# huyhoang17/DB_text_minimal

Hardware: AMD Instinct MI355X
Metric: train images/sec @640x640 bs=16/GPU (higher is better)
Workload: dtype f32

## Files before the change

db_text_minimal_amd/_lib.py:

```python
import ctypes
import os
import subprocess

_HERE = os.path.dirname(os.path.abspath(__file__))
LIB_PATH = os.environ.get('DBN_LIB_PATH') or os.path.join(_HERE, 'libdbnet_hip.so')
CSRC = os.path.join(_HERE, 'csrc')

_P, _I, _L, _F = ctypes.c_void_p, ctypes.c_int, ctypes.c_long, ctypes.c_float

SIGNATURES = {
    'dbn_pack_weights': 'piiiiiipp',
    'dbn_igemm_panel_floats': 'iiiiii',
    'dbn_igemm_packed_floats': 'ii',
    'dbn_igemm_f32': 'pppp' + 'i' * 14 + 'p',
    'dbn_igemm_tile_config': 'ii',
    'dbn_igemm_tile_config_ns': 'iii',
    'dbn_conv_bn_ws_floats': 'iiiiii',
    'dbn_pack_weights_batched': 'piip',
    'dbn_igemm_splitk_plan': 'iiii',
    'dbn_igemm_splitk_plan_ns': 'iiiii',
    'dbn_igemm_splitk_f32': 'pppp' + 'i' * 16 + 'pp',
    'dbn_deform_im2col': 'ppp' + 'i' * 11 + 'p',
    'dbn_deform_col2im': 'ppppp' + 'i' + 'p' + 'i' * 11 + 'p',
    'dbn_deform_col2im_ws_bytes': 'i' * 8,
# ... 82 lines not shown
    'dbn_db_loss_fwd': 'pp' + 'iiii' + 'ffff' + 'pppp',
    'dbn_db_loss_sum_fwd': 'pp' + 'iiii' + 'ffff' + 'pppp',
    'dbn_db_loss_frac_fwd': 'pp' + 'iiii' + 'ffff' + 'i' + 'pppp',
    'dbn_db_loss_bwd': 'pppp' + 'ff' + 'iiii' + 'pp',
    'dbn_db_loss_ohem_ws_bytes': 'iii',
    'dbn_db_loss_ohem_fwd': 'pp' + 'iiii' + 'ffff' + 'pppp',
    'dbn_db_loss_ohem_bwd': 'ppppp' + 'ff' + 'iiii' + 'pp',
    'dbn_pixel_confusion': 'plppiiifpp',
    'dbn_adam_step': 'pppp' + 'l' + 'ffff' + 'i' + 'f' + 'p',
    'dbn_clock_probe': 'pip',
    'dbn_has_experiments': '',
    'dbn_wall_clock_khz': '',
}
SIGNATURES.update({
    'dbn_igemm_t': 'ii' + 'pppp' + 'i' * 14 + 'i' + 'p' + 'p',
    'dbn_conv_bn_t': 'i' + SIGNATURES['dbn_conv_bn_f32'],
    'dbn_pyramid_conv_t': 'i' + SIGNATURES['dbn_pyramid_conv_f32'],
    'dbn_pyramid_conv_from_t': 'ii' + SIGNATURES['dbn_pyramid_conv_f32'],
    'dbn_igemm_bn_rows': 'i' * 15,
    'dbn_igemm_bnsums_t': 'ii' + 'pppp' + 'i' * 14 + 'ppppppp' + 'pppp' + 'p' + 'p',
    'dbn_igemm_bn_final_counters': 'ii',
    'dbn_igemm_bn_final_group_floats': 'ii',
    'dbn_wgrad_t': 'ii' + 'pppp' + 'i' * 12 + 'f' + 'p',
    'dbn_wgrad_phase_t': 'iii' + 'pppp' + 'i' * 12 + 'f' + 'p',
    'dbn_wgrad_reduce_describe': 'ii' + 'pppp' + 'i' * 12 + 'f' + 'p',
    'dbn_wgrad_reduce_many': 'ppiiip',
    'dbn_wgrad_tile_config': 'ii',
    'dbn_set_wgrad_variant': 'i',
    'dbn_set_convt_kernel': 'i',
    'dbn_igemm_splitk_slab_floats': 'iiiii',
    'dbn_wgrad_kernel_config': 'iiiii',
    'dbn_wgrad_kernel_config_hw': 'i' * 12,
    'dbn_set_patch_conv': 'i',
    'dbn_set_wres16': 'i',
    'dbn_set_pyramid_wide': 'i',
    'dbn_pyramid_wide_would_run': 'iiiiii',
    'dbn_conv_bn_set_final': 'pp',
    'dbn_conv_bn_final_group_doubles': 'ii',
    'dbn_wres16_would_run': 'iiiiiiiii',
    'dbn_mfma_sustained': 'ippip',
    'dbn_mfma_sustained_flops': 'ii',
    'dbn_set_stagger': 'i',
    'dbn_winograd_eligible': 'iiiii',
    'dbn_winograd_panel_floats': 'ii',
    'dbn_winograd_pack': 'piiiipp',
    'dbn_winograd_rows': 'iii',
    'dbn_winograd_pack_batched': 'pip',
    'dbn_winograd_dgrad_bnsums_f32': 'ppp' + 'iiiiii' + 'pppp' + 'ppp' + 'pppp' + 'p' + 'p',
    'dbn_winograd_ws_floats': 'iiii',
    'dbn_winograd_wgrad_eligible': 'iiiiii',
    'dbn_winograd_wgrad_linear': 'ii',
    'dbn_winograd_wgrad_slab_floats': 'iiiii',
    'dbn_winograd_wgrad_f32': 'ipppppp' + 'iiiiii' + 'fp',
    'dbn_winograd_conv_bn_act_f32': 'pppppp' + 'iiiii' + 'pp' + 'ff' + 'ppppppp' + 'p',
    'dbn_winograd_conv_bn_f32': 'pppp' + 'iiiii' + 'pp' + 'ff' + 'ppppppp' + 'p',
    'dbn_set_phase_priority': 'i',
    'dbn_set_winograd_persistent': 'i',
    'dbn_set_winograd_stagger': 'i',
    'dbn_set_winograd_blocks_per_barrier': 'i',
    'dbn_fold_bn_eval': 'pilppppp' + 'f' + 'ppp',
    'dbn_igemm_act_t': 'ii' + 'pppp' + 'i' + 'p' + 'i' * 13 + 'p',
    'dbn_winograd_conv_act_f32': 'pppp' + 'i' + 'p' + 'iiiii' + 'p',
    'dbn_pyramid_conv_act_t': 'ii' + 'p' * 9 + 'i' + 'p' + 'i' * 6 + 'p',
    'dbn_set_trace': 'pl',
    'dbn_igemm_kernel_config': 'i' * 16,
    'dbn_split3': 'pplp',
    'dbn_deform_im2col_t': 'i' + SIGNATURES['dbn_deform_im2col'],
    'dbn_deform_col2im_t': 'i' + SIGNATURES['dbn_deform_col2im'],
    'dbn_deform_col2im_gather_t': 'i' + SIGNATURES['dbn_deform_col2im'],
    'dbn_deform_col2im_gather_ws_bytes': 'iii',
    'dbn_deform_offset_absmax_t': 'iplpp',
    'dbn_pw16_eligible': 'iiiiii',
    'dbn_pw16_panel_bytes': '',
    'dbn_pw16_pack': 'ipipp',
    'dbn_pw16_act_t': 'ipppipiiiip',
    'dbn_set_head_tail_wide': 'i',
    'dbn_stem16_pool_eligible': 'iiii',
    'dbn_stem16_conv_bn_relu_pool_t': 'ipppppiiip',
    'dbn_head16_eligible': 'iiii',
    'dbn_head16_tail_eval_t': 'i' + 'p' * 15 + 'iii' + 'p',
    'dbn_cast_f32': 'ipplp',
    'dbn_pack_weights_t': 'ip' + 'i' * 7 + 'pp',
    'dbn_igemm_panel_floats_t': 'i' * 8,
    'dbn_bn_train_stats_t': 'i' + SIGNATURES['dbn_bn_train_stats'],
    'dbn_bn_apply_t': 'i' + SIGNATURES['dbn_bn_apply'],
    'dbn_bn_backward_t': 'ipi' + SIGNATURES['dbn_bn_backward_ex'][1:],
    'dbn_col_sum_t': 'i' + SIGNATURES['dbn_col_sum'],
    'dbn_bnrelu_maxpool_fwd_t': 'i' + SIGNATURES['dbn_bnrelu_maxpool_fwd'],
    'dbn_bnrelu_maxpool_bwd_t': 'i' + SIGNATURES['dbn_bnrelu_maxpool_bwd'][:-1] + 'pppp',
    'dbn_maxpool_bwd_parts': 'iiii',
    'dbn_bnrelu_maxpool_fwd_arg_t': 'ipppppp' + 'iiii' + 'p',
    'dbn_maxpool_bn_backward_ws_floats': 'iiii',
    'dbn_maxpool_bn_backward_t': 'i' + 'p' * 10 + 'iiii' + 'f' + 'pp',
    'dbn_nearest_up_fwd_t': 'i' + SIGNATURES['dbn_nearest_up_fwd'],
    'dbn_nearest_up_bwd_t': 'i' + SIGNATURES['dbn_nearest_up_bwd'],
    'dbn_nchw3_to_nhwc4_t': 'i' + SIGNATURES['dbn_nchw3_to_nhwc4'],
    'dbn_nchw3_to_nhwc4_packed_t': 'i' + SIGNATURES['dbn_nchw3_to_nhwc4'],
    'dbn_nchw3_to_nhwc16_and_4_t': 'ipppiiip',
    'dbn_convt16_rows': '',
    'dbn_convt16_panel_bytes': '',
    'dbn_convt16_eligible': 'iiiiii',
    'dbn_convt16_pack': 'ippp',
    'dbn_convt16_bn_t': 'ippppiii' + 'pp' + 'ff' + 'ppppppp' + 'p',
    'dbn_stem16_padded_h': 'i',
    'dbn_stem16_padded_w': 'i',
    'dbn_stem16_rows': '',
# ... 74 lines not shown
```

db_text_minimal_amd/csrc/wgrad.hip:

```cpp
#include "wgrad_kernels.h"

namespace {

constexpr int WRG = 16;
__global__ __launch_bounds__(256) void wgrad_reduce_kernel(const float* __restrict__ slab, int splitk, int O, int J, int Jp, int BM, int BN,
                                                           int Cb, int I, int R, int S, float* __restrict__ grad, float scale, int natural) {
    __shared__ double part[WRG][16][4];
    const long total = (long)O * Jp, count4 = total >> 2, total4 = wgrad_slab_stride(O, Jp) >> 2;
    const int pos = threadIdx.x & 15, g = threadIdx.x >> 4;
    const long q = blockIdx.x * 16L + pos;
    double s[4] = {0.0, 0.0, 0.0, 0.0};
    if (q < count4) {
        const f32x4* src = reinterpret_cast<const f32x4*>(slab) + q;
        int z = g;
        for (; z + 3 * WRG < splitk; z += 4 * WRG) {
            const f32x4 v0 = src[(long)z * total4], v1 = src[(long)(z + WRG) * total4];
            const f32x4 v2 = src[(long)(z + 2 * WRG) * total4], v3 = src[(long)(z + 3 * WRG) * total4];
#pragma unroll
            for (int e = 0; e < 4; ++e) s[e] += ((double)v0[e] + (double)v1[e]) + ((double)v2[e] + (double)v3[e]);
        }
        for (; z < splitk; z += WRG) {
            const f32x4 v = src[(long)z * total4];
#pragma unroll
            for (int e = 0; e < 4; ++e) s[e] += (double)v[e];
// ... 295 lines not shown
        size_t smem;
        wgrad_reduce64_plan(R * S, splits_total, G, threads, smem);
        *reduce_job = WgradReduceJob{slab, grad_oihw, splits_total, O, J, Jp, bm, bn, Cb, I, R * S, G, natural ? 1 : 0, O * (Cb / 64), scale,
                                     (int)smem};
        return DBN_OK;
    }
    if (Cb % 64 == 0 && R * S * 64 * 4 <= 32 * 1024) {
        int G, threads;
        size_t smem;
        wgrad_reduce64_plan(R * S, splits_total, G, threads, smem);
        hipLaunchKernelGGL(wgrad_reduce64_kernel, dim3(O, Cb / 64), dim3(threads), smem, st, slab, splits_total, O, J, Jp, bm, bn, Cb, I,
                           R * S, G, grad_oihw, scale, natural ? 1 : 0);
    } else
        hipLaunchKernelGGL(wgrad_reduce_kernel, dim3((unsigned)(((long)O * Jp / 4 + 15) / 16)), dim3(256), 0, st, slab, splits_total, O, J, Jp, bm, bn,
                           Cb, I, R, S, grad_oihw, scale, natural ? 1 : 0);
    return dbn_status();
}

int dbn_wgrad_t(int at, int ns, const void* sm, const void* big, float* slab, float* grad_oihw, int N, int Ho, int Wo, int O, int H, int W,
                int Cb, int I, int R, int S, int stride, int pad, float scale, void* stream) {
    return wgrad_run(sm, big, slab, grad_oihw, N, Ho, Wo, O, H, W, Cb, I, R, S, stride, pad, scale, ns, stream, at);
}
int dbn_wgrad_phase_t(int phase, int at, int ns, const void* sm, const void* big, float* slab, float* grad_oihw, int N, int Ho, int Wo,
                      int O, int H, int W, int Cb, int I, int R, int S, int stride, int pad, float scale, void* stream) {
    DBN_REQUIRE(phase == 1 || phase == 2);
    return wgrad_run(sm, big, slab, grad_oihw, N, Ho, Wo, O, H, W, Cb, I, R, S, stride, pad, scale, ns, stream, at, phase);
}

int dbn_wgrad_reduce_describe(int at, int ns, const void* sm, const void* big, float* slab, float* grad_oihw, int N, int Ho, int Wo, int O,
                              int H, int W, int Cb, int I, int R, int S, int stride, int pad, float scale, void* job) {
    DBN_REQUIRE(job);
    return wgrad_run(sm, big, slab, grad_oihw, N, Ho, Wo, O, H, W, Cb, I, R, S, stride, pad, scale, ns, nullptr, at, 2,
                     reinterpret_cast<WgradReduceJob*>(job));
}
int dbn_wgrad_reduce_many(const void* jobs, const int* first, int n_jobs, int total_blocks, int max_smem, void* stream) {
    DBN_REQUIRE(jobs && first && n_jobs > 0 && total_blocks > 0 && max_smem > 0 && max_smem <= 64 * 1024);
    hipLaunchKernelGGL(wgrad_reduce64_many_kernel, dim3(total_blocks), dim3(1024), (size_t)max_smem, (hipStream_t)stream,
                       reinterpret_cast<const WgradReduceJob*>(jobs), first, n_jobs);
    return dbn_status();
}

int dbn_wgrad_f32(const float* sm, const float* big, float* slab, float* grad_oihw, int N, int Ho, int Wo, int O, int H, int W,
                  int Cb, int I, int R, int S, int stride, int pad, float scale, void* stream) {
    return wgrad_run(sm, big, slab, grad_oihw, N, Ho, Wo, O, H, W, Cb, I, R, S, stride, pad, scale, 0, stream);
}

int dbn_wgrad_bf16s(const float* sm, const float* big, float* slab, float* grad_oihw, int N, int Ho, int Wo, int O, int H, int W,
                    int Cb, int I, int R, int S, int stride, int pad, float scale, int ns, void* stream) {
    DBN_REQUIRE(ns == 1 || ns == 3);
    return wgrad_run(sm, big, slab, grad_oihw, N, Ho, Wo, O, H, W, Cb, I, R, S, stride, pad, scale, ns, stream);
}

}
```

db_text_minimal_amd/csrc/wgrad_kernels.h:

```cpp
#pragma once
#include "igemm_common.h"

struct WgradParams {
    const void* sm;
    const void* big;
    float* slab;
    int N, Ho, Wo, O, H, W, Cb, R, S, stride, pad;
    int P, J, pchunk;
    float rcp_HWo, rcp_Wo;
    unsigned sm_bytes, big_bytes;
    unsigned sm_plane_bytes, big_plane_bytes;
    int row_tw;
};

static inline int wgrad_row_tw(int Ho, int Wo) { return Wo % 16 == 0 ? 16 : (Wo % 8 == 0 && Ho % 2 == 0) ? 8 : (Wo % 4 == 0 && Ho % 4 == 0) ? 4 : 0; }

#ifndef DBN_DBG
#define DBN_DBG 0
#endif

namespace {

__host__ __device__ inline long wgrad_slab_stride(long O, long Jp) { return O * Jp + 1088; }


__host__ __device__ __forceinline__ int tile_pos_to_index(int pos, int B) { return 4 * (pos % (B / 4)) + pos / (B / 4); }

template <int BM, int BN, int WM, int WN, int NS, int AT = 0, int ROW = 0>
__global__ __launch_bounds__(WM* WN * 64) void wgrad_f32_kernel(const WgradParams p) {
    static_assert(AT == 0 || (AT == 1 && NS == 1) || (AT == 3 && NS == 3), "storage type / matrix math combination");
    static_assert(!ROW || AT == 0, "scalar-offset addressing is built for fp32 storage");
    constexpr unsigned ES = AT == 0 ? 4u : 2u;
    constexpr int NP = AT == 3 ? 3 : 1;
    constexpr int NT = WM * WN * 64;
    constexpr int TM = BM / WM, TN = BN / WN;
    constexpr int MI = TM / 32, NI = TN / 32;
    constexpr int AS = NS == 0 ? BM + 2 : BM + 4, BS = NS == 0 ? BN + 2 : BN + 4;
    constexpr int A_IMG = NS == 0 ? 4 * AS : NS * 2 * AS, B_IMG = NS == 0 ? 4 * BS : NS * 2 * BS;
    constexpr int STAGE = A_IMG + B_IMG;
    constexpr int NSX = NS > 0 ? NS : 1;
    static_assert(BM + BN <= NT && BM % 64 == 0 && BN % 64 == 0, "staging roles must fit the workgroup in whole waves");
    __shared__ f32x4 smem[2 * STAGE];

    const int tid = threadIdx.x;
    const int lane = tid & 63, wave = tid >> 6;
    const int wm = wave / WN, wn = wave % WN;
    const int li = lane & 31, lh = lane >> 5;

    const int njt = (p.J + BN - 1) / BN;
    const int ntiles = (p.O / BM) * njt;
    const int work = dbn_xcd_remap(blockIdx.x, gridDim.x);
    const int split = work / ntiles, tile_ = work - split * ntiles;
    const int ot = tile_ / njt, jt = tile_ - ot * njt;
    const int o0 = ot * BM, j0 = jt * BN;
    const int pbeg = (DBN_DBG & 8) ? 0 : split * p.pchunk;
    const int pend = min(p.P, pbeg + p.pchunk);
    const int KT = (pend - pbeg + 15) / 16;

    const __amdgpu_buffer_rsrc_t rs_sm = __builtin_amdgcn_make_buffer_rsrc(const_cast<void*>(p.sm), 0, p.sm_bytes, 0x00020000);
    const unsigned row_shift = ROW ? (unsigned)((p.pad * p.W + p.pad) * p.Cb) * ES : 0u;
    const __amdgpu_buffer_rsrc_t rs_big = __builtin_amdgcn_make_buffer_rsrc(
        const_cast<char*>(reinterpret_cast<const char*>(p.big) - row_shift), 0, p.big_bytes + row_shift, 0x00020000);

    const int wave_first = __builtin_amdgcn_readfirstlane(tid) & ~63;
    const bool is_a = wave_first < BM;
    const bool is_b = wave_first >= NT - BN;
    const int slot = is_a ? tid : tid - (NT - BN);
    const int qn = is_a ? BM / 4 : BN / 4;
    const int s_c = slot % qn, s_g = slot / qn;
    const int jj = j0 + 4 * s_c;
    const bool j_ok = is_b && jj < p.J;
    const int tap = j_ok ? jj / p.Cb : 0;
    const int ci = j_ok ? jj - tap * p.Cb : 0;
    const int tr = tap / p.S - p.pad, ts = (DBN_DBG & 16) ? 0 : tap % p.S - p.pad;
    const int HWo = p.Ho * p.Wo;
    const int ld = is_a ? AS : BS;
    const int lds_base = (is_a ? 0 : A_IMG) + s_c;

    constexpr int D = AT == 3 ? 1 : NS == 0 ? ((BM == 64 || ROW) ? 2 : 1) : (AT == 0 ? 3 : 4);
    f32x4 rr_[D][4];
    u32x2 rh_[D][NP][4];
    unsigned woff[4] = {OOB_OFFSET, OOB_OFFSET, OOB_OFFSET, OOB_OFFSET};
    int w_n, w_oh, w_ow;
    {
        int rem;
        divmod24(pbeg + 4 * s_g, HWo, p.rcp_HWo, w_n, rem);
        divmod24(rem, p.Wo, p.rcp_Wo, w_oh, w_ow);
    }
    unsigned vcon[4] = {OOB_OFFSET, OOB_OFFSET, OOB_OFFSET, OOB_OFFSET};
    int ccol[4] = {0, 0, 0, 0};
    int crow = 0;
    int s_n = 0, s_oh = 0, s_ow = 0;
    unsigned soff = 0;
    const int TW = ROW ? p.row_tw : 16, TH = 16 / TW;
    if constexpr (ROW) {
        const bool live = KT > 0;
        const int qy = (4 * s_g) / TW;
        crow = qy * p.stride + tr;
#pragma unroll
        for (int i = 0; i < 4; ++i) {
            const int qx = (4 * s_g + i) & (TW - 1);
            if (is_a) {
                vcon[i] = live ? (unsigned)((qy * p.Wo + qx) * p.O + o0 + 4 * s_c) * ES : OOB_OFFSET;
                woff[i] = vcon[i];
            } else if (is_b) {
                ccol[i] = qx * p.stride + ts;
                vcon[i] = (live && j_ok) ? row_shift + (unsigned)((crow * p.W + ccol[i]) * p.Cb + ci) * ES : OOB_OFFSET;
            }
        }
        const int bw = p.Wo / TW, bh = p.Ho / TH;
        const int t0 = __builtin_amdgcn_readfirstlane(pbeg >> 4);
        const int r0 = t0 / bw;
        s_ow = (t0 - r0 * bw) * TW;
        s_n = r0 / bh;
        s_oh = (r0 - s_n * bh) * TH;
// ... 214 lines not shown
    auto step = [&](int kt, auto UU) {
        constexpr int U = decltype(UU)::value;
        const int buf = kt & 1;
        offsets(kt + D);
        issue_loads(UU);
        const f32x4* As = smem + buf * STAGE;
        const f32x4* Bs = As + A_IMG;
        if constexpr (NS == 0) {
            f32x4 af[2][MI], bf[2][NI];
#pragma unroll
            for (int s2 = 0; s2 < 2; ++s2) {
#pragma unroll
                for (int a = 0; a < MI; ++a) af[s2][a] = As[(2 * s2 + lh) * AS + wm * TM + a * 32 + li];
#pragma unroll
                for (int b = 0; b < NI; ++b) bf[s2][b] = Bs[(2 * s2 + lh) * BS + wn * TN + b * 32 + li];
            }
#pragma unroll
            for (int s2 = 0; s2 < 2; ++s2)
#pragma unroll
                for (int e = 0; e < 4; ++e)
#pragma unroll
                    for (int a = 0; a < MI; ++a)
#pragma unroll
                        for (int b = 0; b < NI; ++b)
                            acc[a][b] = __builtin_amdgcn_mfma_f32_32x32x2f32(af[s2][a][e], bf[s2][b][e], acc[a][b], 0, 0, 0);
        } else {
            bf16x8 af[NSX][MI], bf[NSX][NI];
#pragma unroll
            for (int t = 0; t < NS; ++t) {
#pragma unroll
                for (int a = 0; a < MI; ++a) af[t][a] = __builtin_bit_cast(bf16x8, As[(t * 2 + lh) * AS + wm * TM + a * 32 + li]);
#pragma unroll
                for (int b = 0; b < NI; ++b) bf[t][b] = __builtin_bit_cast(bf16x8, Bs[(t * 2 + lh) * BS + wn * TN + b * 32 + li]);
            }
            mfma_split<NS, MI, NI>(af, bf, acc);
        }
        stage(buf ^ 1, std::integral_constant<int, (U + 1) % D>{});
        __syncthreads();
    };
    static_assert(D <= 4, "the k-loop spells the sets out");
    int kt = 0;
    for (; kt + D <= KT; kt += D) {
        step(kt, std::integral_constant<int, 0>{});
        if constexpr (D > 1) step(kt + 1, std::integral_constant<int, 1 % D>{});
        if constexpr (D > 2) step(kt + 2, std::integral_constant<int, 2 % D>{});
        if constexpr (D > 3) step(kt + 3, std::integral_constant<int, 3 % D>{});
    }
    if (kt < KT) step(kt, std::integral_constant<int, 0>{});
    if (D > 2 && kt + 1 < KT) step(kt + 1, std::integral_constant<int, 1 % D>{});
    if (D > 3 && kt + 2 < KT) step(kt + 2, std::integral_constant<int, 2 % D>{});
    }

    const int Jp = njt * BN;
    float* out = p.slab + (long)split * wgrad_slab_stride(p.O, Jp);
#pragma unroll
    for (int a = 0; a < MI; ++a)
#pragma unroll
        for (int b = 0; b < NI; ++b) {
            const int col = j0 + wn * TN + b * 32 + li;
#pragma unroll
            for (int r = 0; r < 16; ++r) {
                const int row = o0 + wm * TM + a * 32 + (r & 3) + 8 * (r >> 2) + 4 * lh;
                out[(long)row * Jp + col] = acc[a][b][r];
            }
        }
}

#if DBN_HAS_EXPERIMENTS
template <int BM, int BN, int WM, int WN>
__global__ __launch_bounds__(256) void wgrad_dma_kernel(const WgradParams p) {
    constexpr int KP = 16;
    constexpr int TM = BM / WM, TN = BN / WN, MI = TM / 32, NI = TN / 32;
    constexpr int A_F4 = KP * BM / 4, B_F4 = KP * BN / 4;
    constexpr int A_INSTR = A_F4 / 64, B_INSTR = B_F4 / 64;
    constexpr int PER_WAVE = (A_INSTR + B_INSTR) / 4;
    static_assert((A_INSTR + B_INSTR) % 4 == 0 && WM * WN == 4, "DMA instructions are dealt to four waves");
    constexpr int NSTG = 3;
    constexpr int STAGE_F4 = A_F4 + B_F4;
    __shared__ f32x4 smem[NSTG * STAGE_F4];

    const int tid = threadIdx.x;
    const int lane = tid & 63;
    const int wave = __builtin_amdgcn_readfirstlane(tid >> 6);
    const int wm = wave / WN, wn = wave % WN;
    const int li = lane & 31, lh = lane >> 5;

    const int njt = (p.J + BN - 1) / BN;
    const int ntiles = (p.O / BM) * njt;
    const int work = dbn_xcd_remap(blockIdx.x, gridDim.x);
    const int split = work / ntiles, tile_ = work - split * ntiles;
    const int ot = tile_ / njt, jt = tile_ - ot * njt;
    const int o0 = ot * BM, j0 = jt * BN;
    const int pbeg = split * p.pchunk;
    const int pend = min(p.P, pbeg + p.pchunk);
    const int KT = (pend - pbeg + KP - 1) / KP;

    const __amdgpu_buffer_rsrc_t rs_sm = __builtin_amdgcn_make_buffer_rsrc(const_cast<void*>(p.sm), 0, p.sm_bytes, 0x00020000);
    const __amdgpu_buffer_rsrc_t rs_big = __builtin_amdgcn_make_buffer_rsrc(const_cast<void*>(p.big), 0, p.big_bytes, 0x00020000);

    const int HWo = p.Ho * p.Wo;
    unsigned a_off[PER_WAVE];
    int a_px[PER_WAVE];
    int b_n[PER_WAVE], b_oh[PER_WAVE], b_ow[PER_WAVE], b_px[PER_WAVE], b_ci[PER_WAVE], b_tr[PER_WAVE], b_ts[PER_WAVE];
    bool b_ok[PER_WAVE];
#pragma unroll
    for (int i = 0; i < PER_WAVE; ++i) {
        const int t = wave * PER_WAVE + i;
// ... 405 lines not shown
#pragma unroll
                    for (int b = 0; b < 3; ++b) asm volatile("" : "+v"(fb[t][b][h2]));
                }
            typedef unsigned u32x4_ __attribute__((ext_vector_type(4)));
            bf16x8 af[NS][1], bf[NS][3];
#pragma unroll
            for (int t = 0; t < NS; ++t) {
                af[t][0] = __builtin_bit_cast(bf16x8, u32x4_{fa[t][0][0], fa[t][0][1], fa[t][1][0], fa[t][1][1]});
#pragma unroll
                for (int b = 0; b < 3; ++b)
                    bf[t][b] = __builtin_bit_cast(bf16x8, u32x4_{fb[t][b][0][0], fb[t][b][0][1], fb[t][b][1][0], fb[t][b][1][1]});
            }
            f32x16 (&acc2)[1][3] = reinterpret_cast<f32x16 (&)[1][3]>(acc);
            mfma_split<NS, 1, 3>(af, bf, acc2);
        });
    }

    float* out = p.slab + (long)split * wgrad_slab_stride(p.O, p.J);
#pragma unroll
    for (int b = 0; b < 3; ++b) {
        const int cblk = 3 * wn + b, s_ = cblk >> 1, half = cblk & 1;
        const int col = (3 * r + s_) * p.Cb + ci0 + 32 * half + li;
#pragma unroll
        for (int e = 0; e < 16; ++e) {
            const int row = o0 + 32 * wm + (e & 3) + 8 * (e >> 2) + 4 * lh;
            out[(long)row * p.J + col] = acc[b][e];
        }
    }
}

template <int NS, int AT, int ROW>
int launch_wgrad_tiles_row(const WgradParams& p, int bm, int bn, dim3 grid, hipStream_t st) {
    if (bn == 192)
        hipLaunchKernelGGL((wgrad_f32_kernel<64, 192, 2, 2, NS, AT, ROW>), grid, dim3(256), 0, st, p);
    else if (bm == 128 && bn == 128)
        hipLaunchKernelGGL((wgrad_f32_kernel<128, 128, 2, 2, NS, AT, ROW>), grid, dim3(256), 0, st, p);
    else if (bn == 128)
        hipLaunchKernelGGL((wgrad_f32_kernel<64, 128, 2, 2, NS, AT, ROW>), grid, dim3(256), 0, st, p);
    else
        hipLaunchKernelGGL((wgrad_f32_kernel<64, 64, 2, 2, NS, AT, ROW>), grid, dim3(256), 0, st, p);
    return dbn_status();
}
template <int NS, int AT>
int launch_wgrad_tiles(const WgradParams& p, int bm, int bn, dim3 grid, hipStream_t st) {
    if constexpr (AT == 0)
        if (p.row_tw && p.pchunk % 16 == 0) return launch_wgrad_tiles_row<NS, AT, 1>(p, bm, bn, grid, st);
    return launch_wgrad_tiles_row<NS, AT, 0>(p, bm, bn, grid, st);
}

}

int dbn_launch_wgrad_f32(const WgradParams& p, int kind, int bm, int bn, dim3 grid, hipStream_t st);
int dbn_launch_wgrad_b16(const WgradParams& p, int kind, int ns, int at, int bm, int bn, dim3 grid, hipStream_t st);
```

db_text_minimal_amd/csrc/winograd_wgrad_f32.hip:

```cpp
#include "igemm_common.h"
#include <algorithm>
#ifndef DBN_WWG_PIPE
#define DBN_WWG_PIPE 1
#endif
#ifndef DBN_WWG_EXP
#define DBN_WWG_EXP 0
#endif

namespace {

constexpr int WG_XPX = 180, WG_XROW = 18, WG_YPX = 128, WG_YROW = 16;

struct WinoWgradParams {
    const float* x;
    const float* dy;
    float* slab;
    int N, H, W, Cx, Cy;
    int nob, nib;
    int tw, gpi, groups;
    int nsplit;
    unsigned x_bytes, dy_bytes;
    const float *x_scale, *x_shift;
};

constexpr int WL_XPX = 336, WL_YPX = 240;
template <bool LIN>
__global__ __launch_bounds__(512) __attribute__((amdgpu_waves_per_eu(2, 2))) void winograd_wgrad_f32_kernel(const WinoWgradParams p) {
    constexpr int XPX = LIN ? WL_XPX : WG_XPX, YPX = LIN ? WL_YPX : WG_YPX;
    constexpr int XCH = XPX * 16, YCH = YPX * 16;
    constexpr int NXP = (XCH + 511) / 512, NYP = (YCH + 511) / 512;
    constexpr int NBUF = LIN ? 1 : 2;
    __shared__ f32x4 smem[NBUF * (XCH + YCH)];
    const int tid = threadIdx.x, lane = tid & 63, wave = __builtin_amdgcn_readfirstlane(tid >> 6);
    const int li = lane & 31, lh = lane >> 5;
    const int irow = wave & 3, oh = wave >> 2;
    const int nsub = p.nob * p.nib;
    const int b = dbn_xcd_remap(blockIdx.x, gridDim.x);
    const int split = b / nsub, sub = b - split * nsub;
    const int ob = sub / p.nib, ib = sub - ob * p.nib;
    const int g0 = (int)((long)split * p.groups / p.nsplit), g1 = (int)((long)(split + 1) * p.groups / p.nsplit);
    const __amdgpu_buffer_rsrc_t rsX = __builtin_amdgcn_make_buffer_rsrc(const_cast<float*>(p.x), 0, p.x_bytes, 0x00020000);
    const __amdgpu_buffer_rsrc_t rsY = __builtin_amdgcn_make_buffer_rsrc(const_cast<float*>(p.dy), 0, p.dy_bytes, 0x00020000);
    const int TW = (p.W + 1) >> 1, TI = ((p.H + 1) >> 1) * TW;
    const int prow = LIN ? 2 * TW + 2 : WG_XROW, yrow = LIN ? 2 * TW : WG_YROW;
    const float rTW = 1.0f / (float)TW;

    unsigned xrel[NXP], yrel[NYP];
    int xpos[NXP], ypos[NYP];
#pragma unroll
    for (int j = 0; j < NXP; ++j) {
        const int idx = tid + j * 512, pix = idx >> 4, ch = idx & 15;
        int py, px;
        if constexpr (LIN) divmod24(pix, prow, 1.0f / (float)prow, py, px);
// ... 327 lines not shown
    for (int pt = 0; pt < 16; ++pt)
#pragma unroll
        for (int e = 0; e < 4; ++e) acc[pt][e] = 0.0;
    for (int z = z0; z < z1; ++z) {
        f32x4 v[16];
#pragma unroll
        for (int pt = 0; pt < 16; ++pt) v[pt] = *reinterpret_cast<const f32x4*>(src + z * stride + pt * 4096);
#pragma unroll
        for (int pt = 0; pt < 16; ++pt)
#pragma unroll
            for (int e = 0; e < 4; ++e) acc[pt][e] += (double)v[pt][e];
    }
    if (zl2 >= ZH) {
#pragma unroll
        for (int pt = 0; pt < 16; ++pt)
#pragma unroll
            for (int e = 0; e < 4; ++e) part[zl * OG + og][pt][iq * 4 + e] = acc[pt][e];
    }
    __syncthreads();
    if (zl2 < ZH) {
#pragma unroll
        for (int pt = 0; pt < 16; ++pt)
#pragma unroll
            for (int e = 0; e < 4; ++e) part[zl * OG + og][pt][iq * 4 + e] += acc[pt][e];
    }
    __syncthreads();
    for (int k = threadIdx.x; k < OG * 16 * 32; k += 256) {
        const int g = k >> 9, pt = (k >> 5) & 15, c = k & 31;
        double s_ = 0.0;
#pragma unroll
        for (int q = 0; q < ZH; ++q) s_ += part[q * OG + g][pt][c];
        sh[g][pt][c] = s_;
    }
    __syncthreads();
    for (int k = threadIdx.x; k < OG * 288; k += 256) {
        const int g = k / 288, kk = k - g * 288, c = kk / 9, tap = kk - c * 9, r = tap / 3, q = tap - r * 3;
        auto gcol = [](int w, double v0, double v1, double v2, double v3) {
            return w == 0 ? v0 + 0.5 * (v1 + v2) : (w == 1 ? 0.5 * (v1 - v2) : 0.5 * (v1 + v2) + v3);
        };
        double t[4];
#pragma unroll
        for (int i = 0; i < 4; ++i) t[i] = gcol(q, sh[g][4 * i + 0][c], sh[g][4 * i + 1][c], sh[g][4 * i + 2][c], sh[g][4 * i + 3][c]);
        st[k] = (float)(gcol(r, t[0], t[1], t[2], t[3]) * (double)scale);
    }
    __syncthreads();
    const int c0 = ib * 64 + ih * 32;
    const int n = max(0, min(32, I - c0)) * 9;
    for (int k = threadIdx.x; k < OG * n; k += 256) {
        const int g = k / n, kk = k - g * n;
        grad[((long)(blockIdx.x * OG + g) * I + c0) * 9 + kk] = st[g * 288 + kk];
    }
}

int wwg_splits(int groups, int nsub) {
    static const int wgs = dbn_env_int("DBN_WWG_WGS", 256);
    int ns = std::max(1, wgs / nsub);
    return std::min(ns, groups);
}

bool wwg_linear_fits(int H, int W) {
    const int TW = (W + 1) / 2, TH = (H + 1) / 2;
    const int R = std::min(TH, (30 + TW) / TW + 1);
    return (2 * R + 2) * (2 * TW + 2) <= WL_XPX && 2 * R * 2 * TW <= WL_YPX;
}
double wwg_fill(int H, int W, bool lin) {
    if (lin) {
        const long TI = (long)((H + 1) / 2) * ((W + 1) / 2);
        return (double)TI / (double)((TI + 31) / 32 * 32);
    }
    return (double)H * W / ((double)((H + 7) / 8 * 8) * ((W + 15) / 16 * 16));
}
bool wwg_linear(int H, int W) {
    static const int env = dbn_env_int("DBN_WWG_LIN", 1);
    return env && wwg_linear_fits(H, W) && wwg_fill(H, W, true) > wwg_fill(H, W, false) + 0.2;
}
int wwg_groups(int N, int H, int W) {
    if (wwg_linear(H, W)) return N * (int)(((long)((H + 1) / 2) * ((W + 1) / 2) + 31) / 32);
    return N * ((H + 7) / 8) * ((W + 15) / 16);
}

}

extern "C" {

int dbn_winograd_wgrad_eligible(int N, int H, int W, int O, int Cb, int I) {
    if (N < 1 || H < 1 || W < 1 || O % 64 || Cb % 64 || I < 1 || I > Cb) return 0;
    const long px = (long)N * H * W;
    if (px * std::max(O, Cb) * 4 >= dbn_g_byte_limit) return 0;
    return wwg_fill(H, W, wwg_linear(H, W)) >= 0.5;
}
int dbn_winograd_wgrad_linear(int H, int W) { return wwg_linear(H, W); }
long dbn_winograd_wgrad_slab_floats(int N, int H, int W, int O, int Cb) {
    const int nsub = (O / 64) * (Cb / 64);
    return (long)wwg_splits(wwg_groups(N, H, W), nsub) * nsub * 16 * 4096;
}
int dbn_winograd_wgrad_f32(int phases, const float* dy, const float* x, const float* x_scale, const float* x_shift, float* slab, float* grad,
                           int N, int H, int W, int O, int Cb, int I, float scale, void* stream) {
    DBN_REQUIRE(dy && x && slab && grad && phases >= 1 && phases <= 3 && !x_scale == !x_shift);
    DBN_REQUIRE(dbn_winograd_wgrad_eligible(N, H, W, O, Cb, I));
    WinoWgradParams p;
    p.x = x;
    p.dy = dy;
    p.slab = slab;
    p.x_scale = x_scale;
    p.x_shift = x_shift;
    p.N = N;
    p.H = H;
    p.W = W;
    p.Cx = Cb;
    p.Cy = O;
    p.nob = O / 64;
    p.nib = Cb / 64;
    const bool lin = wwg_linear(H, W);
    p.tw = (W + 15) / 16;
    p.groups = wwg_groups(N, H, W);
    p.gpi = p.groups / N;
    p.nsplit = wwg_splits(p.groups, p.nob * p.nib);
    p.x_bytes = (unsigned)((long)N * H * W * Cb * 4);
    p.dy_bytes = (unsigned)((long)N * H * W * O * 4);
    hipStream_t st = (hipStream_t)stream;
    if (phases & 1) {
        const dim3 grid(p.nsplit * p.nob * p.nib);
        if (lin) hipLaunchKernelGGL(winograd_wgrad_f32_kernel<true>, grid, dim3(512), 0, st, p);
        else hipLaunchKernelGGL(winograd_wgrad_f32_kernel<false>, grid, dim3(512), 0, st, p);
    }
    if (phases & 2) {
        const int nsub = p.nob * p.nib;
        if (p.nsplit >= 128)
            hipLaunchKernelGGL(winograd_wgrad_reduce_kernel<32>, dim3(O, 2 * p.nib), dim3(256), 0, st, slab, p.nsplit, nsub, p.nib, I, grad, scale);
        else
            hipLaunchKernelGGL(winograd_wgrad_reduce_serial_kernel, dim3(O, p.nib), dim3(1024), 0, st, slab, p.nsplit, nsub, p.nib, I, grad, scale);
    }
    return dbn_status();
}

}
```

include/dbnet_hip.h:

```cpp
#ifndef DBNET_HIP_H
#define DBNET_HIP_H
#ifdef __cplusplus
extern "C" {
#endif


int dbn_pack_weights(const float* w_oihw, int O, int I, int R, int S, int mode, int stride, float* out, void* stream);
long dbn_igemm_panel_floats(int O, int I, int R, int S, int mode, int stride);
int dbn_igemm_packed_floats(int K, int Cd);

int dbn_igemm_f32(const float* src, const float* wpk, const float* bias, float* dst, int N, int Hs, int Ws, int Cs, int Hd,
                  int Wd, int Cd, int R, int S, int stride, int pad, int mode, int accumulate, int tile_hint, void* stream);

int dbn_pack_weights_bf16s(const float* w_oihw, int O, int I, int R, int S, int mode, int stride, int ns, float* out, void* stream);
int dbn_pack_weights_batched(const void* jobs, int n, int ns, void* stream);
long dbn_igemm_bf16s_panel_floats(int O, int I, int R, int S, int mode, int stride, int ns);
int dbn_igemm_bf16s(const float* src, const float* wpk, const float* bias, float* dst, int N, int Hs, int Ws, int Cs, int Hd,
                    int Wd, int Cd, int R, int S, int stride, int pad, int mode, int accumulate, int tile_hint, int ns,
                    void* stream);
int dbn_wgrad_bf16s(const float* sm, const float* big, float* slab, float* grad_oihw, int N, int Ho, int Wo, int O, int H, int W,
                    int Cb, int I, int R, int S, int stride, int pad, float scale, int ns, void* stream);

int dbn_igemm_bn_rows(int at, int ns, int N, int Hs, int Ws, int Cs, int Hd, int Wd, int Cd, int R, int S, int stride, int pad, int mode,
                      int tile_hint);
// ... 82 lines not shown
                           float* dz, int N, int H, int W, int C, void* stream);

int dbn_nearest_up_fwd(const float* src, const float* addend, float* dst, int N, int Hs, int Ws, int C, int H, int W, int Cdst,
                       int coff, void* stream);
int dbn_nearest_up_bwd(const float* dbig, float* dsrc, int N, int Hs, int Ws, int C, int H, int W, int Cbig, int coff,
                       int accumulate, void* stream);

int dbn_bilinear_fwd(const float* src, float* dst, long planes, int Hs, int Ws, int H, int W, void* stream);
int dbn_bilinear_bwd(const float* ddst, float* dsrc, long planes, int Hs, int Ws, int H, int W, void* stream);

int dbn_fpn_combine_weights(const float* w, int Co, int Cin, int group, int Cg, float* wd, void* stream);
int dbn_fpn_scatter_wgrad(const float* t0, const float* t1, const float* t2, const float* t3, int Co, int Cg, float* dw,
                          void* stream);

int dbn_nchw3_to_nhwc4(const float* x, float* out, int N, int H, int W, void* stream);
int dbn_add_inplace(const float* x, float* y, long n, void* stream);

int dbn_head_tail_fwd(const float* xb, const float* xt, const float* wb, const float* wt, const float* bias_b,
                      const float* bias_t, const float* bn_scale_b, const float* bn_shift_b, const float* bn_scale_t,
                      const float* bn_shift_t, float* out, int N, int Hq, int Wq, int channels, float kstep, void* stream);
int dbn_head_tail_bwd_ws_floats(void);
int dbn_head_tail_bwd(const float* xb, const float* xt, const float* wb, const float* wt, const float* preds,
                      const float* dpreds, const float* bn_scale_b, const float* bn_shift_b, const float* bn_scale_t,
                      const float* bn_shift_t, const float* bn_mean_b, const float* bn_rstd_b, const float* bn_mean_t,
                      const float* bn_rstd_t, float* bn_sums, float* dxb, float* dxt, float* dw_b, float* dbias_b, float* dw_t,
                      float* dbias_t, int N, int Hq, int Wq, int channels, float kstep, float grad_scale, float* ws, void* stream);

int dbn_set_winograd_persistent(int on);
int dbn_set_winograd_stagger(int permille);
int dbn_set_winograd_blocks_per_barrier(int n);
int dbn_winograd_eligible(int N, int H, int W, int Cs, int Cd);
long dbn_winograd_panel_floats(int O, int Cs);
int dbn_winograd_pack(const float* w_oihw, int O, int I, int Cs, int dgrad, float* out, void* stream);
int dbn_winograd_pack_batched(const void* jobs, int n, void* stream);
int dbn_winograd_rows(int N, int H, int W);
int dbn_winograd_dgrad_bnsums_f32(const float* dy, const float* upanel, float* dx, int N, int H, int W, int Cs, int Cd, int accumulate,
                                  const void* y, const void* zmask, const float* mask_scale, const float* mask_shift,
                                  const float* save_mean, const float* save_rstd, float* part, const void* y2, const float* save_mean2,
                                  const float* save_rstd2, float* part2, const dbn_bnb_final* fin, void* stream);
long dbn_winograd_ws_floats(int N, int H, int W, int Cd);
int dbn_winograd_conv_bn_act_f32(const float* src, const float* in_scale, const float* in_shift, const float* upanel, const float* bias,
                                 float* dst, int N, int H, int W, int Cs, int Cd, const float* gamma, const float* beta, float eps,
                                 float momentum, float* run_mean, float* run_var, float* scale, float* shift, float* save_mean,
                                 float* save_rstd, float* ws, void* stream);
int dbn_winograd_conv_bn_f32(const float* src, const float* upanel, const float* bias, float* dst, int N, int H, int W, int Cs, int Cd,
                             const float* gamma, const float* beta, float eps, float momentum, float* run_mean, float* run_var,
                             float* scale, float* shift, float* save_mean, float* save_rstd, float* ws, void* stream);

int dbn_winograd_wgrad_eligible(int N, int H, int W, int O, int Cb, int I);
int dbn_winograd_wgrad_linear(int H, int W);
long dbn_winograd_wgrad_slab_floats(int N, int H, int W, int O, int Cb);
int dbn_winograd_wgrad_f32(int phases, const float* dy, const float* x, const float* x_scale, const float* x_shift, float* slab, float* grad,
                           int N, int H, int W, int O, int Cb, int I, float scale, void* stream);

int dbn_db_loss_ws_bytes(void);
int dbn_db_loss_fwd(const float* preds, const float* gts, int N, int H, int W, int channels, float alpha, float beta,
                    float negative_ratio, float eps, float* losses, float* coef, void* ws, void* stream);
int dbn_db_loss_bwd(const float* preds, const float* gts, const float* coef, const float* grad_losses, float alpha, float beta,
                    int N, int H, int W, int channels, float* dpreds, void* stream);
int dbn_db_loss_sum_fwd(const float* preds, const float* gts, int N, int H, int W, int channels, float alpha, float beta,
                        float negative_ratio, float eps, float* losses, float* coef, void* ws, void* stream);
int dbn_db_loss_frac_fwd(const float* preds, const float* gts, int N, int H, int W, int channels, float alpha, float beta,
                         float negative_ratio, float eps, int sum, float* losses, float* coef, void* ws, void* stream);

long dbn_db_loss_ohem_ws_bytes(int N, int H, int W);
int dbn_db_loss_ohem_fwd(const float* preds, const float* gts, int N, int H, int W, int channels, float alpha, float beta,
                         float negative_ratio, float eps, float* losses, float* coef, void* ws, void* stream);
int dbn_db_loss_ohem_bwd(const float* preds, const float* gts, const float* coef, const float* grad_losses, const void* ws,
                         float alpha, float beta, int N, int H, int W, int channels, float* dpreds, void* stream);

int dbn_pixel_confusion(const float* preds, long batch_stride, const float* gt, const float* mask, int N, int H, int W, float thresh,
                        double* hist, void* stream);

int dbn_adam_step(float* p, const float* g, float* m, float* v, long n, float lr, float beta1, float beta2, float eps, int step,
                  float grad_scale, void* stream);

int dbn_has_experiments(void);

int dbn_clock_probe(void* out2, int microseconds, void* stream);
int dbn_wall_clock_khz(void);

int dbn_deform_im2col(const float* x, const float* offset, float* cols, int N, int H, int W, int C, int Ho, int Wo, int R, int S,
                      int stride, int pad, int off_stride, void* stream);
long dbn_deform_col2im_ws_bytes(int N, int H, int W, int C, int Ho, int Wo, int R, int S);
int dbn_deform_col2im(const float* dcols, const float* x, const float* offset, float* dx, float* doffset, int accumulate, void* ws, int N,
                      int H, int W, int C, int Ho, int Wo, int R, int S, int stride, int pad, int off_stride, void* stream);
int dbn_permute_weight(const float* src, float* dst, int O, int C, int T, int to_ohwi, float scale, void* stream);

int dbn_binarize_u8(const float* pred, int N, int channels, int H, int W, float thresh, unsigned char* out, void* stream);
int dbn_box_scores(const float* bitmap, int H, int W, const float* boxes, int K, int P, float* scores, void* stream);

int dbn_gt_maps(const double* verts, const double* dist, const int* meta, const int* img_off, const int* ixy, int N, int P, int S,
                int max_verts, int max_off_pts, float scale, float tmin, float* out, void* stream);
int dbn_normalize_u8(const unsigned char* in, int N, int H, int W, float m0, float m1, float m2, float* out, void* stream);
int dbn_poly_offset(const double* xy, int n, const double* delta, int* out_xy, int cap, int* out_n);
int dbn_poly_offset_paths(const double* xy, int n, const double* delta, int* out_xy, int cap, int* out_n, int* out_paths);

int dbn_warp_affine_u8(const unsigned char* src, long src_bytes, const long long* desc, const double* coef, int N, int max_h, int max_w,
                       unsigned char* dst, long dst_bytes, void* stream);
int dbn_resize_cubic_u8(const unsigned char* src, long src_bytes, const long long* desc, const double* coef, int N, int max_h, int max_w,
                        unsigned char* dst, long dst_bytes, void* stream);
int dbn_resize_linear_norm_u8(const unsigned char* src, long src_bytes, const long long* desc, const double* coef, int N, int CH, int CW,
                              float m0, float m1, float m2, float* out, void* stream);

int dbn_perspective_maps(const float* quads, int K, int out_h, int out_w, double* fwd, double* inv);
int dbn_warp_perspective_u8(const unsigned char* src, long src_bytes, const long long* desc, const double* inv, int K, int out_h, int out_w,
// ... 219 lines not shown
```

Before: 724.3.

## Add transform-domain Winograd weight-gradient path using batched GEMM over 16 planes

Adds an alternative Winograd wgrad path that first transforms input tiles and output-gradient tiles into 16 transform-domain planes in global memory. It then runs the existing f32 wgrad GEMM kernel batched over those planes via blockIdx.z. A final kernel reduces the split-K partials and applies the inverse filter transform to produce 3x3 weight gradients. The aim is to replace the fused Winograd wgrad kernel with more regular batched GEMMs when the transformed buffers fit a size budget. The cost is extra workspace and memory traffic for the intermediate transformed tensors, plus a heuristic that chooses between the two paths.

```diff
diff --git a/db_text_minimal_amd/_lib.py b/db_text_minimal_amd/_lib.py
--- a/db_text_minimal_amd/_lib.py
+++ b/db_text_minimal_amd/_lib.py
@@ -158,6 +158,7 @@
     'dbn_winograd_wgrad_linear': 'ii',
     'dbn_winograd_wgrad_slab_floats': 'iiiii',
     'dbn_winograd_wgrad_f32': 'ipppppp' + 'iiiiii' + 'fp',
+    'dbn_set_winograd_wgrad_path': 'ii',
     'dbn_winograd_conv_bn_act_f32': 'pppppp' + 'iiiii' + 'pp' + 'ff' + 'ppppppp' + 'p',
     'dbn_winograd_conv_bn_f32': 'pppp' + 'iiiii' + 'pp' + 'ff' + 'ppppppp' + 'p',
     'dbn_set_phase_priority': 'i',
diff --git a/db_text_minimal_amd/csrc/wgrad.hip b/db_text_minimal_amd/csrc/wgrad.hip
--- a/db_text_minimal_amd/csrc/wgrad.hip
+++ b/db_text_minimal_amd/csrc/wgrad.hip
@@ -371,3 +371,41 @@
 }
 
 }
+
+WgradBatchPlan dbn_wgrad_batch_plan(int batch, int P, int O, int Cb, int force_splits) {
+    WgradBatchPlan pl;
+    wgrad_tiles(O, Cb, pl.bm, pl.bn);
+    const int njt = (Cb + pl.bn - 1) / pl.bn;
+    pl.Jp = njt * pl.bn;
+    const long wgs = (long)batch * (O / pl.bm) * njt;
+    long sk = force_splits > 0 ? force_splits : std::max(1L, std::min(256 / wgs, (long)P / 64));
+    sk = std::max(1L, std::min(sk, ((long)P + 15) / 16));
+    pl.pchunk = (int)((((long)P + sk - 1) / sk + 15) / 16 * 16);
+    pl.splitk = (P + pl.pchunk - 1) / pl.pchunk;
+    pl.slab_batch = (long)pl.splitk * wgrad_slab_stride(O, pl.Jp);
+    pl.slab_floats = (long)batch * pl.slab_batch;
+    return pl;
+}
+
+int dbn_launch_wgrad_batch_f32(const float* sm, const float* big, float* slab, int batch, int P, int O, int Cb, const WgradBatchPlan& pl,
+                               hipStream_t st) {
+    DBN_REQUIRE(sm && big && slab && batch >= 1 && batch <= 65535 && P >= 1 && (long)P < dbn_g_pixel_limit - 64 && O % 64 == 0 && Cb % 4 == 0);
+    DBN_REQUIRE((long)P * std::max(O, Cb) * 4 < dbn_g_byte_limit);
+    WgradParams p;
+    p.sm = sm; p.big = big; p.slab = slab;
+    p.N = 1; p.Ho = 1; p.Wo = P; p.O = O; p.H = 1; p.W = P; p.Cb = Cb; p.R = 1; p.S = 1; p.stride = 1; p.pad = 0;
+    p.P = P;
+    p.J = Cb;
+    p.pchunk = pl.pchunk;
+    p.rcp_HWo = 1.0f / (float)P;
+    p.rcp_Wo = 1.0f / (float)P;
+    p.sm_bytes = (unsigned)((long)P * O * 4);
+    p.big_bytes = (unsigned)((long)P * Cb * 4);
+    p.sm_plane_bytes = p.big_plane_bytes = 0;
+    p.row_tw = g_wgrad_row16 ? wgrad_row_tw(1, P) : 0;
+    p.sm_batch = (long)P * O * 4;
+    p.big_batch = (long)P * Cb * 4;
+    p.slab_batch = pl.slab_batch;
+    const dim3 grid((O / pl.bm) * (pl.Jp / pl.bn) * pl.splitk, 1, batch);
+    return dbn_launch_wgrad_f32(p, 0, pl.bm, pl.bn, grid, st);
+}
diff --git a/db_text_minimal_amd/csrc/wgrad_kernels.h b/db_text_minimal_amd/csrc/wgrad_kernels.h
--- a/db_text_minimal_amd/csrc/wgrad_kernels.h
+++ b/db_text_minimal_amd/csrc/wgrad_kernels.h
@@ -11,6 +11,7 @@
     unsigned sm_bytes, big_bytes;
     unsigned sm_plane_bytes, big_plane_bytes;
     int row_tw;
+    long sm_batch = 0, big_batch = 0, slab_batch = 0;
 };
 
 static inline int wgrad_row_tw(int Ho, int Wo) { return Wo % 16 == 0 ? 16 : (Wo % 8 == 0 && Ho % 2 == 0) ? 8 : (Wo % 4 == 0 && Ho % 4 == 0) ? 4 : 0; }
@@ -57,10 +58,12 @@
     const int pend = min(p.P, pbeg + p.pchunk);
     const int KT = (pend - pbeg + 15) / 16;
 
-    const __amdgpu_buffer_rsrc_t rs_sm = __builtin_amdgcn_make_buffer_rsrc(const_cast<void*>(p.sm), 0, p.sm_bytes, 0x00020000);
+    const long zb = blockIdx.z;
+    const __amdgpu_buffer_rsrc_t rs_sm = __builtin_amdgcn_make_buffer_rsrc(
+        const_cast<char*>(reinterpret_cast<const char*>(p.sm) + zb * p.sm_batch), 0, p.sm_bytes, 0x00020000);
     const unsigned row_shift = ROW ? (unsigned)((p.pad * p.W + p.pad) * p.Cb) * ES : 0u;
     const __amdgpu_buffer_rsrc_t rs_big = __builtin_amdgcn_make_buffer_rsrc(
-        const_cast<char*>(reinterpret_cast<const char*>(p.big) - row_shift), 0, p.big_bytes + row_shift, 0x00020000);
+        const_cast<char*>(reinterpret_cast<const char*>(p.big) + zb * p.big_batch - row_shift), 0, p.big_bytes + row_shift, 0x00020000);
 
     const int wave_first = __builtin_amdgcn_readfirstlane(tid) & ~63;
     const bool is_a = wave_first < BM;
@@ -381,7 +384,7 @@
     }
 
     const int Jp = njt * BN;
-    float* out = p.slab + (long)split * wgrad_slab_stride(p.O, Jp);
+    float* out = p.slab + zb * p.slab_batch + (long)split * wgrad_slab_stride(p.O, Jp);
 #pragma unroll
     for (int a = 0; a < MI; ++a)
 #pragma unroll
@@ -893,3 +896,11 @@
 
 int dbn_launch_wgrad_f32(const WgradParams& p, int kind, int bm, int bn, dim3 grid, hipStream_t st);
 int dbn_launch_wgrad_b16(const WgradParams& p, int kind, int ns, int at, int bm, int bn, dim3 grid, hipStream_t st);
+
+struct WgradBatchPlan {
+    int bm, bn, Jp, splitk, pchunk;
+    long slab_batch, slab_floats;
+};
+WgradBatchPlan dbn_wgrad_batch_plan(int batch, int P, int O, int Cb, int force_splits);
+int dbn_launch_wgrad_batch_f32(const float* sm, const float* big, float* slab, int batch, int P, int O, int Cb, const WgradBatchPlan& plan,
+                               hipStream_t st);
diff --git a/db_text_minimal_amd/csrc/winograd_wgrad_f32.hip b/db_text_minimal_amd/csrc/winograd_wgrad_f32.hip
--- a/db_text_minimal_amd/csrc/winograd_wgrad_f32.hip
+++ b/db_text_minimal_amd/csrc/winograd_wgrad_f32.hip
@@ -1,4 +1,4 @@
-#include "igemm_common.h"
+#include "wgrad_kernels.h"
 #include <algorithm>
 #ifndef DBN_WWG_PIPE
 #define DBN_WWG_PIPE 1
@@ -432,6 +432,132 @@
     }
 }
 
+__device__ __forceinline__ double wwg_gcol(int k, double v0, double v1, double v2, double v3) {
+    return k == 0 ? v0 + 0.5 * (v1 + v2) : (k == 1 ? 0.5 * (v1 - v2) : 0.5 * (v1 + v2) + v3);
+}
+__device__ __forceinline__ int wwg_row(int t) {
+    const int q = (t >> 1) & 7, k = t & 1;
+    return (t & ~15) + 8 * (q >> 2) + 4 * k + (q & 3);
+}
+__global__ __launch_bounds__(256) void winograd_wgrad_xform_x_kernel(const float* __restrict__ x, const float* __restrict__ x_scale,
+                                                                     const float* __restrict__ x_shift, float* __restrict__ V, int N, int H,
+                                                                     int W, int C, int TH, int TW) {
+    const int cq = C >> 2;
+    const long T = (long)N * TH * TW, Tp = (T + 15) & ~15L, idx = (long)blockIdx.x * 256 + threadIdx.x;
+    if (idx >= Tp * cq) return;
+    const int tile = (int)(idx / cq), q = (int)(idx - (long)tile * cq);
+    const bool real = tile < T;
+    const int n = tile / (TH * TW), tr = tile - n * (TH * TW), ty = tr / TW, tx = tr - ty * TW;
+    const bool act = x_scale != nullptr;
+    f32x4 sc = {0.f, 0.f, 0.f, 0.f}, shv = {0.f, 0.f, 0.f, 0.f};
+    if (act) {
+        sc = reinterpret_cast<const f32x4*>(x_scale)[q];
+        shv = reinterpret_cast<const f32x4*>(x_shift)[q];
+    }
+    f32x4 d[4][4];
+#pragma unroll
+    for (int a = 0; a < 4; ++a)
+#pragma unroll
+        for (int b = 0; b < 4; ++b) {
+            const int h = 2 * ty - 1 + a, w = 2 * tx - 1 + b;
+            const bool in = real && (unsigned)h < (unsigned)H && (unsigned)w < (unsigned)W;
+            f32x4 v = {0.f, 0.f, 0.f, 0.f};
+            if (in) {
+                v = reinterpret_cast<const f32x4*>(x + (((long)n * H + h) * W + w) * C)[q];
+                if (act) {
+#pragma unroll
+                    for (int e = 0; e < 4; ++e) v[e] = dbn_affine_relu(v[e], sc[e], shv[e]);
+                }
+            }
+            d[a][b] = v;
+        }
+    f32x4* const out = reinterpret_cast<f32x4*>(V) + (long)wwg_row(tile) * cq + q;
+    const long plane = Tp * cq;
+#pragma unroll
+    for (int i = 0; i < 4; ++i) {
+        f32x4 R[4];
+#pragma unroll
+        for (int b = 0; b < 4; ++b) R[b] = i == 0 ? d[0][b] - d[2][b] : (i == 1 ? d[1][b] + d[2][b] : (i == 2 ? d[2][b] - d[1][b] : d[1][b] - d[3][b]));
+        out[(4 * i + 0) * plane] = R[0] - R[2];
+        out[(4 * i + 1) * plane] = R[1] + R[2];
+        out[(4 * i + 2) * plane] = R[2] - R[1];
+        out[(4 * i + 3) * plane] = R[1] - R[3];
+    }
+}
+__global__ __launch_bounds__(256) void winograd_wgrad_xform_dy_kernel(const float* __restrict__ dy, float* __restrict__ D, int N, int H, int W,
+                                                                      int C, int TH, int TW) {
+    const int cq = C >> 2;
+    const long T = (long)N * TH * TW, Tp = (T + 15) & ~15L, idx = (long)blockIdx.x * 256 + threadIdx.x;
+    if (idx >= Tp * cq) return;
+    const int tile = (int)(idx / cq), q = (int)(idx - (long)tile * cq);
+    const bool real = tile < T;
+    const int n = tile / (TH * TW), tr = tile - n * (TH * TW), ty = tr / TW, tx = tr - ty * TW;
+    f32x4 y[2][2];
+#pragma unroll
+    for (int a = 0; a < 2; ++a)
+#pragma unroll
+        for (int b = 0; b < 2; ++b) {
+            const int h = 2 * ty + a, w = 2 * tx + b;
+            f32x4 v = {0.f, 0.f, 0.f, 0.f};
+            if (real && h < H && w < W) v = reinterpret_cast<const f32x4*>(dy + (((long)n * H + h) * W + w) * C)[q];
+            y[a][b] = v;
+        }
+    f32x4* const out = reinterpret_cast<f32x4*>(D) + (long)wwg_row(tile) * cq + q;
+    const long plane = Tp * cq;
+#pragma unroll
+    for (int i = 0; i < 4; ++i) {
+        f32x4 r[2];
+#pragma unroll
+        for (int b = 0; b < 2; ++b) r[b] = i == 0 ? y[0][b] : (i == 1 ? y[0][b] + y[1][b] : (i == 2 ? y[0][b] - y[1][b] : -y[1][b]));
+        out[(4 * i + 0) * plane] = r[0];
+        out[(4 * i + 1) * plane] = r[0] + r[1];
+        out[(4 * i + 2) * plane] = r[0] - r[1];
+        out[(4 * i + 3) * plane] = -r[1];
+    }
+}
+__global__ __launch_bounds__(256) void winograd_wgrad_output_kernel(const float* __restrict__ slab, int splitk, long slab_batch, int O, int Jp,
+                                                                    int BM, int BN, int I, float* __restrict__ grad, float scale) {
+    __shared__ double sh[16][192];
+    __shared__ float st[192 * 9];
+    const int o = blockIdx.x, jt = blockIdx.y, om = o % BM;
+    const int prow = (o / BM) * BM + (om & 3) * (BM / 4) + (om >> 2);
+    const long sstride = wgrad_slab_stride(O, Jp);
+    const int nq = BN >> 2;
+    for (int w = threadIdx.x; w < 16 * nq; w += 256) {
+        const int pt = w / nq, q = w - pt * nq;
+        const float* src = slab + pt * slab_batch + (long)prow * Jp + jt * BN + 4 * q;
+        double s[4] = {0.0, 0.0, 0.0, 0.0};
+        int z = 0;
+        for (; z + 3 < splitk; z += 4) {
+            const f32x4 v0 = *reinterpret_cast<const f32x4*>(src + z * sstride), v1 = *reinterpret_cast<const f32x4*>(src + (z + 1) * sstride);
+            const f32x4 v2 = *reinterpret_cast<const f32x4*>(src + (z + 2) * sstride), v3 = *reinterpret_cast<const f32x4*>(src + (z + 3) * sstride);
+#pragma unroll
+            for (int e = 0; e < 4; ++e) s[e] += ((double)v0[e] + (double)v1[e]) + ((double)v2[e] + (double)v3[e]);
+        }
+        for (; z < splitk; ++z) {
+            const f32x4 v = *reinterpret_cast<const f32x4*>(src + z * sstride);
+#pragma unroll
+            for (int e = 0; e < 4; ++e) s[e] += (double)v[e];
+        }
+#pragma unroll
+        for (int e = 0; e < 4; ++e) sh[pt][4 * q + e] = s[e];
+    }
+    __syncthreads();
+    for (int k = threadIdx.x; k < BN * 9; k += 256) {
+        const int c = k / 9, tap = k - c * 9, r = tap / 3, q = tap - r * 3;
+        const int pos = (c & 3) * (BN / 4) + (c >> 2);
+        double t[4];
+#pragma unroll
+        for (int i = 0; i < 4; ++i) t[i] = wwg_gcol(q, sh[4 * i + 0][pos], sh[4 * i + 1][pos], sh[4 * i + 2][pos], sh[4 * i + 3][pos]);
+        st[k] = (float)(wwg_gcol(r, t[0], t[1], t[2], t[3]) * (double)scale);
+    }
+    __syncthreads();
+    const int c0 = jt * BN;
+    const int n = max(0, min(BN, I - c0)) * 9;
+    float* dst = grad + ((long)o * I + c0) * 9;
+    for (int k = threadIdx.x; k < n; k += 256) dst[k] = st[k];
+}
+
 int wwg_splits(int groups, int nsub) {
     static const int wgs = dbn_env_int("DBN_WWG_WGS", 256);
     int ns = std::max(1, wgs / nsub);
@@ -459,25 +585,85 @@
     return N * ((H + 7) / 8) * ((W + 15) / 16);
 }
 
+int g_wwg_path = 0;
+int g_wwg_splits = 0;
+constexpr long WWG_TD_BYTES = 110L << 20;
+long wwg_tiles(int N, int H, int W) { return (long)N * ((H + 1) / 2) * ((W + 1) / 2); }
+long wwg_rows(int N, int H, int W) { return (wwg_tiles(N, H, W) + 15) / 16 * 16; }
+bool wwg_tdomain_can(int N, int H, int W, int O, int Cb) {
+    const long T = wwg_rows(N, H, W);
+    return T < dbn_g_pixel_limit - 64 && T * std::max(O, Cb) * 4 < dbn_g_byte_limit;
+}
+int wwg_td_splits(int N, int H, int W, int O, int Cb) {
+    if (g_wwg_splits > 0) return g_wwg_splits;
+    if (!wwg_linear(H, W)) return 0;
+    const int TI = ((H + 1) / 2) * ((W + 1) / 2), gpi = (TI + 31) / 32, groups = N * gpi;
+    const int ns = wwg_splits(groups, (O / 64) * (Cb / 64));
+    if (ns >= 128 || groups % ns || (groups / ns) % gpi || TI % 2) return 0;
+    const long rows = (long)(groups / ns / gpi) * TI;
+    return rows % 16 == 0 ? ns : 0;
+}
+WgradBatchPlan wwg_td_plan(int N, int H, int W, int O, int Cb) {
+    return dbn_wgrad_batch_plan(16, (int)wwg_rows(N, H, W), O, Cb, wwg_td_splits(N, H, W, O, Cb));
+}
+bool wwg_tdomain(int N, int H, int W, int O, int Cb) {
+    if (g_wwg_path == 1 || !wwg_tdomain_can(N, H, W, O, Cb)) return false;
+    if (g_wwg_path == 2) return true;
+    const long T = wwg_rows(N, H, W);
+    const WgradBatchPlan pl = dbn_wgrad_batch_plan(16, (int)T, O, Cb, 0);
+    return 16 * T * (Cb + O) * 4 <= WWG_TD_BYTES && 16L * (O / pl.bm) * (pl.Jp / pl.bn) >= 256 && g_wwg_splits == 0 &&
+           wwg_td_splits(N, H, W, O, Cb) > 0;
+}
 }
 
 extern "C" {
 
+static bool wwg_valid(int N, int H, int W, int O, int Cb, int I) {
+    if (N < 1 || H < 1 || W < 1 || O < 64 || O % 64 || Cb < 64 || Cb % 64 || I < 1 || I > Cb) return false;
+    const long px = (long)N * H * W;
+    return px * std::max(O, Cb) * 4 < dbn_g_byte_limit;
+}
 int dbn_winograd_wgrad_eligible(int N, int H, int W, int O, int Cb, int I) {
-    if (N < 1 || H < 1 || W < 1 || O % 64 || Cb % 64 || I < 1 || I > Cb) return 0;
-    const long px = (long)N * H * W;
-    if (px * std::max(O, Cb) * 4 >= dbn_g_byte_limit) return 0;
+    if (!wwg_valid(N, H, W, O, Cb, I)) return 0;
     return wwg_fill(H, W, wwg_linear(H, W)) >= 0.5;
 }
 int dbn_winograd_wgrad_linear(int H, int W) { return wwg_linear(H, W); }
 long dbn_winograd_wgrad_slab_floats(int N, int H, int W, int O, int Cb) {
+    if (wwg_tdomain(N, H, W, O, Cb)) {
+        return 16 * wwg_rows(N, H, W) * (Cb + O) + wwg_td_plan(N, H, W, O, Cb).slab_floats;
+    }
     const int nsub = (O / 64) * (Cb / 64);
     return (long)wwg_splits(wwg_groups(N, H, W), nsub) * nsub * 16 * 4096;
+}
+int dbn_set_winograd_wgrad_path(int path, int splits) {
+    DBN_REQUIRE(path >= 0 && path <= 2 && splits >= 0);
+    g_wwg_path = path;
+    g_wwg_splits = splits;
+    return DBN_OK;
 }
 int dbn_winograd_wgrad_f32(int phases, const float* dy, const float* x, const float* x_scale, const float* x_shift, float* slab, float* grad,
                            int N, int H, int W, int O, int Cb, int I, float scale, void* stream) {
     DBN_REQUIRE(dy && x && slab && grad && phases >= 1 && phases <= 3 && !x_scale == !x_shift);
-    DBN_REQUIRE(dbn_winograd_wgrad_eligible(N, H, W, O, Cb, I));
+    DBN_REQUIRE(wwg_valid(N, H, W, O, Cb, I));
+    if (wwg_tdomain(N, H, W, O, Cb)) {
+        hipStream_t st = (hipStream_t)stream;
+        const int TH = (H + 1) / 2, TW = (W + 1) / 2, T = (int)wwg_rows(N, H, W);
+        const WgradBatchPlan pl = wwg_td_plan(N, H, W, O, Cb);
+        float* const V = slab;
+        float* const D = V + 16L * T * Cb;
+        float* const dU = D + 16L * T * O;
+        if (phases & 1) {
+            hipLaunchKernelGGL(winograd_wgrad_xform_x_kernel, dim3((unsigned)(((long)T * (Cb / 4) + 255) / 256)), dim3(256), 0, st, x, x_scale,
+                               x_shift, V, N, H, W, Cb, TH, TW);
+            hipLaunchKernelGGL(winograd_wgrad_xform_dy_kernel, dim3((unsigned)(((long)T * (O / 4) + 255) / 256)), dim3(256), 0, st, dy, D, N, H, W,
+                               O, TH, TW);
+            if (const int rc = dbn_launch_wgrad_batch_f32(D, V, dU, 16, T, O, Cb, pl, st)) return rc;
+        }
+        if (phases & 2)
+            hipLaunchKernelGGL(winograd_wgrad_output_kernel, dim3(O, pl.Jp / pl.bn), dim3(256), 0, st, dU, pl.splitk, pl.slab_batch, O, pl.Jp,
+                               pl.bm, pl.bn, I, grad, scale);
+        return dbn_status();
+    }
     WinoWgradParams p;
     p.x = x;
     p.dy = dy;
diff --git a/include/dbnet_hip.h b/include/dbnet_hip.h
--- a/include/dbnet_hip.h
+++ b/include/dbnet_hip.h
@@ -158,6 +158,7 @@
 long dbn_winograd_wgrad_slab_floats(int N, int H, int W, int O, int Cb);
 int dbn_winograd_wgrad_f32(int phases, const float* dy, const float* x, const float* x_scale, const float* x_shift, float* slab, float* grad,
                            int N, int H, int W, int O, int Cb, int I, float scale, void* stream);
+int dbn_set_winograd_wgrad_path(int path, int splits);
 
 int dbn_db_loss_ws_bytes(void);
 int dbn_db_loss_fwd(const float* preds, const float* gts, int N, int H, int W, int channels, float alpha, float beta,
```

After: 733.9 (median of 6 runs). 1.01x the previous value.
